# ttwang0303/Adaptive-RGBD-Localization-Mappig

Measured on AMD Instinct MI355X. Metric: frames/sec (extract+match+RANSAC-PnP) @640x480, 2000 kp, higher is better.
Workload: dtype u8/i32 (extract, match), f32+f64 (ransac, pnp)

## Files before the change

adaptive-rgbd-localization-mappig_amd/csrc/k_extract.hip:

```cpp
#include "odo_device.h"
#include "odo_internal.h"
#include "odo_wave.h"
#ifdef FS_STATS
#include <cstdio>
#endif

#ifndef ODO_EXTRACT_PRIO
#define ODO_EXTRACT_PRIO 0
#endif
#define EXTRACT_PRIO() \
    if (ODO_EXTRACT_PRIO) __builtin_amdgcn_s_setprio(ODO_EXTRACT_PRIO)

namespace odo {

__global__ void __launch_bounds__(256) k_gray(const uint8_t* __restrict__ bgr, uint8_t* __restrict__ pyr,
                                              int w, int h, int pitch, size_t in_stride, size_t pyr_stride) {
    EXTRACT_PRIO();
    const int f = blockIdx.y;
    const int q = blockIdx.x * blockDim.x + threadIdx.x;
    const uint8_t* src = bgr + (size_t)f * in_stride;
    uint8_t* dst = pyr + (size_t)f * pyr_stride;
    const int npix = w * h;
    const int p0 = q * 4;
    if (p0 >= npix) return;
// ... 1414 lines not shown
            const int src = reflect101_1(x - 4 + 4 * d + bb, L.w) - (x - 4);
            const int sd = src >> 2, sb = src & 3;
            a |= (uint32_t)(sd == 0 ? sb : sd == 1 ? 4 + sb : 0x0c) << (8 * bb);
            bsel |= (uint32_t)(sd == 2 ? sb : 0x0c) << (8 * bb);
        }
        selA[d] = a;
        selB[d] = bsel;
    }
    const int o0 = x >= 4 ? x - 4 : x, o2 = x + 8 <= L.pitch ? x + 4 : x;
    const uint8_t* s0 = srcL;
    uint8_t* dp = blur + (size_t)f * pyr_stride + L.off + (size_t)y0 * L.pitch + x;
    blur_walk<true, BR_RE>(s0, dp, (size_t)L.pitch, L.h, y0, true, true, true, o0, x, o2, selA, selB);
}

__global__ void __launch_bounds__(256) k_blur_rows(const uint8_t* __restrict__ pyr, uint8_t* __restrict__ blur,
                                                   size_t pyr_stride, const LevelDesc* __restrict__ lv, BlurRows S,
                                                   int nlevels, int eblocks) {
    EXTRACT_PRIO();
    const int f = blockIdx.y;
    if ((int)blockIdx.x < eblocks) {
        const int k = (int)blockIdx.x * 256 + (int)threadIdx.x;
        if (k >= S.ebase[nlevels]) return;
        int l = 0;
        while (l + 1 < nlevels && k >= S.ebase[l + 1]) l++;
        blur_edge_lane(pyr + (size_t)f * pyr_stride + lv[l].off, blur, pyr_stride, lv, S, nlevels, f, k);
        return;
    }
    const uint32_t none[3] = {0, 0, 0};
    const int item = ((int)blockIdx.x - eblocks) * 16 + ((int)threadIdx.x >> 4);
    if (item >= S.base[nlevels]) return;
    int l = 0;
    while (l + 1 < nlevels && item >= S.base[l + 1]) l++;
    const LevelDesc L = lv[l];
    const int it = item - S.base[l];
    const int chunk = it / S.nst[l], strip = it - chunk * S.nst[l];
    const int q = 1 + strip * 16 + ((int)threadIdx.x & 15);
    const bool store = q <= S.nq[l];
    const int x = 4 * (store ? q : S.nq[l]);
    const int y0 = chunk_y0<BR_R>(chunk, L.h);
    const bool top = y0 < 3, bottom = y0 + BR_R + 3 > L.h;
    const uint8_t* s0 = pyr + (size_t)f * pyr_stride + L.off + (x - 4);
    uint8_t* dp = blur + (size_t)f * pyr_stride + L.off + (size_t)y0 * L.pitch + x;
    blur_walk<false, BR_R>(s0, dp, (size_t)L.pitch, L.h, y0, top, bottom, store, 0, 0, 0, none, none);
}

#ifndef PYR_TH
#define PYR_TH 512
#endif
#ifndef PYR_VGPR
#define PYR_ATTR
#else
#define PYR_ATTR __attribute__((amdgpu_waves_per_eu(PYR_VGPR)))
#endif
#ifndef PYR_RU
#define PYR_RU 4
#endif
#ifndef PYR_GU
#define PYR_GU 8
#endif
struct PyrLevels {
    int rx_off[16], ry_off[16];
};
#ifndef PYR_PARTS
#define PYR_PARTS 1
#endif
struct PyrSplit {
    int parts;
    int lo[2][16], hi[2][16], ca[2][16], cb[2][16], ea[2][16], eb[2][16];
};
ODO_INLINE void pyr_blur_level(const uint8_t* srcL, uint8_t* __restrict__ blur, size_t pyr_stride,
                               const LevelDesc* __restrict__ lv, const BlurRows& S, int nlevels, int f, int l,
                               const LevelDesc& L, int t, int ca, int cb, int ea, int eb) {
    const uint32_t none[3] = {0, 0, 0};
    const int items = cb * S.nst[l];
    const int g = t >> 4;
    for (int it = ca * S.nst[l] + g; it < items; it += PYR_TH / 16) {
        const int chunk = it / S.nst[l], strip = it - chunk * S.nst[l];
        const int q = 1 + strip * 16 + (t & 15);
        const bool store = q <= S.nq[l];
        const int x = 4 * (store ? q : S.nq[l]);
        const int y0 = chunk_y0<BR_R>(chunk, L.h);
        const bool top = y0 < 3, bottom = y0 + BR_R + 3 > L.h;
        const uint8_t* s0 = srcL + (x - 4);
        uint8_t* dp = blur + (size_t)f * pyr_stride + L.off + (size_t)y0 * L.pitch + x;
        blur_walk<false, BR_R>(s0, dp, (size_t)L.pitch, L.h, y0, top, bottom, store, 0, 0, 0, none, none);
    }
    const int ne = (S.ebase[l + 1] - S.ebase[l]) / ((L.h + BR_RE - 1) / BR_RE);
    for (int k = S.ebase[l] + ea * ne + t; k < S.ebase[l] + eb * ne; k += PYR_TH)
        blur_edge_lane(srcL, blur, pyr_stride, lv, S, nlevels, f, k);
}
ODO_INLINE void pyr_resize_rows(const uint8_t* srcS, uint8_t* dstD, const LevelDesc& S, const LevelDesc& D,
                                const ResizeX* __restrict__ X, const ResizeY* __restrict__ Y, int t, int ylo, int yhi) {
    const int nq = (D.w + 3) >> 2;
    const int P = PYR_TH / nq;
    if (t >= P * nq) return;
    const int ph = t / nq, q = t - ph * nq;
    const int x00 = X[4 * q].sx0;
    const int wb = x00 & ~3, sh = x00 & 3;
    uint32_t sel[4], wt[4];
#pragma unroll
    for (int j = 0; j < 4; j++) {
        const int dx = 4 * q + j;
        if (dx < D.w) {
            const ResizeX xj = X[dx];
            const uint32_t r0 = (uint32_t)(xj.sx0 - x00), r1 = (uint32_t)(xj.sx1 - x00);
            sel[j] = r0 | (0x0cu << 8) | (r1 << 16) | (0x0cu << 24);
            wt[j] = (uint32_t)xj.a0 | ((uint32_t)xj.a1 << 16);
        } else {
            sel[j] = 0x0c0c0c0cu;
            wt[j] = 0;
        }
    }
    const uint8_t* sbase = srcS + wb;
    uint8_t* dbase = dstD + 4 * q;
    auto hsum = [&](const uint8_t* row, uint32_t (&h)[4]) {
        const uint32_t* w32 = reinterpret_cast<const uint32_t*>(row);
        const uint32_t w0 = w32[0], w1 = w32[1], w2 = w32[2];
        const uint32_t A = __builtin_amdgcn_alignbyte(w1, w0, sh), B = __builtin_amdgcn_alignbyte(w2, w1, sh);
#pragma unroll
        for (int j = 0; j < 4; j++) {
            typedef unsigned short u16x2 __attribute__((ext_vector_type(2)));
            h[j] = __builtin_amdgcn_udot2(__builtin_bit_cast(u16x2, __builtin_amdgcn_perm(B, A, sel[j])),
                                          __builtin_bit_cast(u16x2, wt[j]), 0u, false);
        }
    };
    for (int y = ylo + ph; y < yhi; y += PYR_RU * P) {
        ResizeY Yr[PYR_RU];
#pragma unroll
        for (int u = 0; u < PYR_RU; u++) Yr[u] = Y[min(y + u * P, yhi - 1)];
        uint32_t h0[PYR_RU][4], h1[PYR_RU][4];
#pragma unroll
        for (int u = 0; u < PYR_RU; u++) {
            hsum(sbase + Yr[u].sy0 * S.pitch, h0[u]);
            hsum(sbase + Yr[u].sy1 * S.pitch, h1[u]);
        }
#pragma unroll
        for (int u = 0; u < PYR_RU; u++) {
            uint32_t pk = 0;
#pragma unroll
            for (int j = 0; j < 4; j++)
                pk |= min((__umul24(h0[u][j], (uint32_t)Yr[u].b0) + __umul24(h1[u][j], (uint32_t)Yr[u].b1) + (1u << 21)) >> 22,
                          255u) << (8 * j);
            if (y + u * P < yhi) *reinterpret_cast<uint32_t*>(dbase + (size_t)(y + u * P) * D.pitch) = pk;
        }
    }
}
ODO_INLINE void pyr_gray_rows(const uint8_t* __restrict__ src, uint8_t* gdst, int w, int pitch, int r0, int r1,
                              int t) {
    if ((w & 3) == 0) {
        const int nq4 = (r1 * w) >> 2;
        const int q00 = ((r0 * w) >> 2) + t;
        int cy = (4 * q00) / w, cx = 4 * q00 - cy * w;
        const int dy = (4 * PYR_TH) / w, dx = 4 * PYR_TH - dy * w;
        for (int q0 = q00; q0 < nq4; q0 += PYR_GU * PYR_TH) {
            uint32_t wv[PYR_GU][3];
#pragma unroll
            for (int u = 0; u < PYR_GU; u++) {
                const int q = q0 + u * PYR_TH;
                if (q < nq4) {
                    const uint32_t* s32 = reinterpret_cast<const uint32_t*>(src + (size_t)q * 12);
                    wv[u][0] = s32[0], wv[u][1] = s32[1], wv[u][2] = s32[2];
                }
            }
#pragma unroll
            for (int u = 0; u < PYR_GU; u++) {
                const int q = q0 + u * PYR_TH;
                const int y = cy, x = cx;
                cx += dx;
                cy += dy;
                if (cx >= w) cx -= w, cy++;
                if (q < nq4) {
                    uint32_t out = 0;
#pragma unroll
                    for (int i = 0; i < 4; i++) {
                        const int b = 3 * i;
                        const uint32_t B = (wv[u][b >> 2] >> (8 * (b & 3))) & 0xffu;
                        const uint32_t G = (wv[u][(b + 1) >> 2] >> (8 * ((b + 1) & 3))) & 0xffu;
                        const uint32_t R = (wv[u][(b + 2) >> 2] >> (8 * ((b + 2) & 3))) & 0xffu;
                        out |= ((B * 1868u + G * 9617u + R * 4899u + 8192u) >> 14) << (8 * i);
                    }
                    *reinterpret_cast<uint32_t*>(gdst + (size_t)y * pitch + x) = out;
                }
            }
        }
    } else {
        for (int p = r0 * w + t; p < r1 * w; p += PYR_TH) {
            const uint8_t* s = src + (size_t)p * 3;
            const int yy = p / w, xx = p - yy * w;
            gdst[(size_t)yy * pitch + xx] =
                (uint8_t)(((uint32_t)s[0] * 1868u + (uint32_t)s[1] * 9617u + (uint32_t)s[2] * 4899u + 8192u) >> 14);
        }
    }
}
template <bool BLUR>
__global__ void __launch_bounds__(PYR_TH) PYR_ATTR k_pyramid(const uint8_t* __restrict__ bgr, uint8_t* __restrict__ pyr,
                                                    size_t in_stride, size_t pyr_stride,
                                                    const LevelDesc* __restrict__ lv, const ResizeX* __restrict__ xt,
                                                    const ResizeY* __restrict__ yt, PyrLevels PL, int nlevels,
                                                    uint8_t* __restrict__ blur, BlurRows BR, PyrSplit SP) {
    EXTRACT_PRIO();
    const int part = SP.parts == 2 ? (int)(blockIdx.x & 1) : 0;
    const int f = SP.parts == 2 ? (int)(blockIdx.x >> 1) : (int)blockIdx.x;
    const int t = threadIdx.x;
    uint8_t* base = pyr + (size_t)f * pyr_stride;
    if (bgr) {
        const LevelDesc L0 = lv[0];
        pyr_gray_rows(bgr + (size_t)f * in_stride, base + L0.off, L0.w, L0.pitch, SP.lo[part][0], SP.hi[part][0], t);
    }
    for (int l = 1; l < nlevels; l++) {
        __syncthreads();
        const LevelDesc S = lv[l - 1], D = lv[l];
        if (BLUR)
            pyr_blur_level(base + S.off, blur, pyr_stride, lv, BR, nlevels, f, l - 1, S, t, SP.ca[part][l - 1],
                           SP.cb[part][l - 1], SP.ea[part][l - 1], SP.eb[part][l - 1]);
        pyr_resize_rows(base + S.off, base + D.off, S, D, xt + PL.rx_off[l], yt + PL.ry_off[l], t, SP.lo[part][l],
                        SP.hi[part][l]);
    }
    if (BLUR) {
        __syncthreads();
        const int ll = nlevels - 1;
        const LevelDesc L = lv[ll];
        pyr_blur_level(base + L.off, blur, pyr_stride, lv, BR, nlevels, f, ll, L, t, SP.ca[part][ll], SP.cb[part][ll],
                       SP.ea[part][ll], SP.eb[part][ll]);
    }
    __syncthreads();
}

}

namespace odo {
void launch_gray(hipStream_t st, const uint8_t* bgr, uint8_t* pyr, int w, int h, int pitch, size_t in_stride,
                 size_t pyr_stride, int nframes) {
    dim3 g((w * h / 4 + 255) / 256 + 1, nframes);
    hipLaunchKernelGGL(k_gray, g, dim3(256), 0, st, bgr, pyr, w, h, pitch, in_stride, pyr_stride);
}
static bool blur_rows_plan(const LevelDesc* lv_host, int nlevels, BlurRows& R) {
    bool rows = nlevels <= 16;
    for (int l = 0; l < nlevels; l++) rows = rows && lv_host[l].h >= BR_R && lv_host[l].w >= 12;
    if (!rows) return false;
    R = BlurRows{};
    int acc = 0, eacc = 0;
    for (int l = 0; l < nlevels; l++) {
        const LevelDesc& L = lv_host[l];
        R.base[l] = acc;
        R.ebase[l] = eacc;
        R.nq[l] = (L.w - 8) / 4;
        R.nst[l] = (R.nq[l] + 15) / 16;
        R.nch[l] = (L.h + BR_R - 1) / BR_R;
        acc += R.nst[l] * R.nch[l];
        eacc += (1 + (L.w + 3) / 4 - (R.nq[l] + 1)) * ((L.h + BR_RE - 1) / BR_RE);
    }
    R.base[nlevels] = acc;
    R.ebase[nlevels] = eacc;
    return true;
}
bool pyramid_blur_fusable(const LevelDesc* lv_host, int nlevels) {
    BlurRows R;
    return blur_rows_plan(lv_host, nlevels, R);
}
static void pyramid_split_plan(const LevelDesc* lv_host, const ResizeY* ry_h, const int* ry_off, int nlevels,
                               int parts, PyrSplit& S) {
    S = PyrSplit{};
    S.parts = parts;
    for (int l = 0; l < nlevels && l < 16; l++) {
        const int h = lv_host[l].h, nch = (h + BR_R - 1) / BR_R, nch6 = (h + BR_RE - 1) / BR_RE;
        for (int p = 0; p < 2; p++) {
            S.lo[p][l] = 0, S.hi[p][l] = h;
            S.ca[p][l] = 0, S.cb[p][l] = nch, S.ea[p][l] = 0, S.eb[p][l] = nch6;
        }
    }
    if (parts != 2 || nlevels > 16 || !ry_h) {
        S.parts = 1;
        return;
    }
    int sp[16];
    for (int l = 0; l < nlevels; l++) {
        const int h = lv_host[l].h;
        int s = ((h / 2 + BR_R / 2) / BR_R) * BR_R;
        if (h < 2 * BR_R) s = h;
        s = std::min(s, h < 2 * BR_R ? h : h - BR_R);
        sp[l] = s;
        const int nch = (h + BR_R - 1) / BR_R, nch6 = (h + BR_RE - 1) / BR_RE;
        S.ca[0][l] = 0, S.cb[0][l] = s == h ? nch : s / BR_R;
        S.ca[1][l] = S.cb[0][l], S.cb[1][l] = nch;
        S.ea[0][l] = 0, S.eb[0][l] = s == h ? nch6 : s / BR_RE;
        S.ea[1][l] = S.eb[0][l], S.eb[1][l] = nch6;
    }
    for (int l = nlevels - 1; l >= 0; l--) {
        const int h = lv_host[l].h;
        int thi = std::min(h, sp[l] + 3), blo = std::max(0, sp[l] - 3);
        if (sp[l] == h) blo = h;
        if (l + 1 < nlevels) {
            const ResizeY* Y = ry_h + ry_off[l + 1];
            if (S.hi[0][l + 1] > 0) thi = std::max(thi, Y[S.hi[0][l + 1] - 1].sy1 + 1);
            if (S.lo[1][l + 1] < lv_host[l + 1].h) blo = std::min(blo, Y[S.lo[1][l + 1]].sy0);
        }
        S.lo[0][l] = 0, S.hi[0][l] = std::min(h, thi);
        S.lo[1][l] = std::max(0, blo), S.hi[1][l] = h;
        if (S.lo[1][l] >= h) S.lo[1][l] = h;
    }
}
void launch_pyramid(hipStream_t st, const uint8_t* bgr, uint8_t* pyr, size_t in_stride, size_t pyr_stride,
                    const LevelDesc* lv, const ResizeX* rx, const ResizeY* ry, const int* rx_off, const int* ry_off,
                    int nlevels, int nframes, uint8_t* blur, const LevelDesc* lv_host, const ResizeY* ry_h) {
    PyrLevels PL{};
    for (int l = 0; l < nlevels && l < 16; l++) PL.rx_off[l] = rx_off[l], PL.ry_off[l] = ry_off[l];
    PyrSplit SP;
    pyramid_split_plan(lv_host, ry_h, ry_off, nlevels, PYR_PARTS, SP);
    const dim3 g(nframes * SP.parts);
    BlurRows BR{};
    if (blur && blur_rows_plan(lv_host, nlevels, BR)) {
        hipLaunchKernelGGL(k_pyramid<true>, g, dim3(PYR_TH), 0, st, bgr, pyr, in_stride, pyr_stride, lv, rx, ry, PL,
                           nlevels, blur, BR, SP);
        return;
    }
    hipLaunchKernelGGL(k_pyramid<false>, g, dim3(PYR_TH), 0, st, bgr, pyr, in_stride, pyr_stride, lv, rx, ry, PL,
                       nlevels, (uint8_t*)nullptr, BR, SP);
}
bool pyramid_fusable(const LevelDesc* lv_host, const ResizeX* rx, const int* rx_off, int nlevels) {
    if (nlevels > 16) return false;
    for (int l = 1; l < nlevels; l++) {
        const LevelDesc& D = lv_host[l];
        const int nq = (D.w + 3) / 4;
        if (nq > PYR_TH) return false;
        const ResizeX* X = rx + rx_off[l];
        for (int q = 0; q < nq; q++) {
            const int x00 = X[4 * q].sx0;
            for (int j = 0; j < 4 && 4 * q + j < D.w; j++) {
                const ResizeX& xj = X[4 * q + j];
                if (xj.sx0 < x00 || xj.sx1 < x00 || xj.sx0 - x00 > 7 || xj.sx1 - x00 > 7) return false;
                if (xj.a0 < 0 || xj.a0 > 65535 || xj.a1 < 0 || xj.a1 > 65535) return false;
            }
        }
    }
    return true;
}
size_t resize_lds_bytes(int spitch, int dw, int max_src_rows) {
    return (size_t)((dw + 3) & ~3) * sizeof(ResizeX) + (size_t)max_src_rows * spitch;
}
void launch_resize(hipStream_t st, uint8_t* pyr, size_t pyr_stride, int src_off, int spitch, int dst_off, int dpitch,
                   int dw, int dh, int rb, int max_src_rows, const ResizeX* xt, const ResizeY* yt, int nframes) {
    dim3 g((dh + rb - 1) / rb, nframes);
    const size_t lds = resize_lds_bytes(spitch, dw, max_src_rows);
    hipLaunchKernelGGL(k_resize, g, dim3(256), lds, st, pyr, pyr_stride, src_off, spitch, dst_off, dpitch, dw, dh, rb,
                       xt, yt);
}
bool fast_lds_plan(const FastSeg* segs, int nsegs, FastLds& L) {
    int img = 16, bw = 1, rows = 1, nl = 1;
    for (int k = 0; k < nsegs; k++) {
        img = std::max(img, (int)segs[k].rows * FS_RS);
        bw = std::max(bw, (int)segs[k].rows * (int)segs[k].bw);
        rows = std::max(rows, (int)segs[k].rows);
        nl = std::max(nl, FS_RS / 4 + FS_NCM);
        if ((int)segs[k].ncell > FS_NCM || (int)segs[k].rows * FS_RS > 65536 || ((segs[k].x0 & 15) + segs[k].cols) > FS_RS)
            return false;
    }
    auto al = [](int x) { return (x + 15) & ~15; };
    L.img = al(img);
    L.ring = 2 * L.img;
    L.clist = L.ring + (FS_TH / 64) * FS_RSTRIDE * 2;
    L.bits = al(L.clist + FS_CL * 2);
    L.cnt = al(L.bits + bw * 4);
    L.qlist = al(L.cnt + rows * FS_NCM * 4);
    L.misc = al(L.qlist + nl * 8);
    L.total = al(L.misc + (int)sizeof(FastMisc));
    return L.total <= 160 * 1024;
}
void launch_fast(hipStream_t st, const uint8_t* pyr, size_t pyr_stride, const FastSeg* segs, int nsegs,
                 const LevelDesc* lv, uint32_t* cand, int* cand_cnt, int ncells, int cell_cap, int ini_th, int min_th,
                 const FastLds& lds, int nframes) {
    static bool attr = false;
    if (!attr) {
        (void)hipFuncSetAttribute((const void*)k_fast_seg, hipFuncAttributeMaxDynamicSharedMemorySize, 160 * 1024);
        attr = true;
    }
    hipLaunchKernelGGL(k_fast_seg, dim3(nsegs, nframes), dim3(FS_TH), lds.total, st, pyr, pyr_stride, segs, lv, cand,
                       cand_cnt, ncells, cell_cap, ini_th, min_th, lds);
#ifdef FS_STATS
    unsigned long long h[8];
    (void)hipStreamSynchronize(st);
    (void)hipMemcpyFromSymbol(h, HIP_SYMBOL(fs_stats), sizeof(h));
    fprintf(stderr, "fs_stats frames %d segs %d items0 %llu items1 %llu survivors %llu segtest_calls %llu corners %llu ovf %llu retry_cells %llu cells %llu\n",
            nframes, nsegs, h[0], h[1], h[2], h[3], h[4], h[5], h[6], h[7]);
    static const unsigned long long z[8] = {};
    (void)hipMemcpyToSymbol(HIP_SYMBOL(fs_stats), z, sizeof(z));
// ... 78 lines not shown
```

adaptive-rgbd-localization-mappig_amd/csrc/odo_batch.cpp:

```cpp
#include "odo_ctx.h"

static int wait_pnp_done(odo_ctx* c, hipStream_t st, int set) {
    if (st != c->pdone_st[set]) HIPCHK(hipStreamWaitEvent(st, c->ev_pnp_done[set], 0));
    return ODO_OK;
}

static int queue_batch_waits(odo_ctx* c) {
    int e;
    const int s = next_set(c);
    if (c->pdone_rec[s] && (e = wait_pnp_done(c, c->stream, s))) return e;
    if (c->batch_counter >= (uint64_t)PYR_WAIT && (e = wait_pnp_done(c, c->stream, (s + NSETS - PYR_WAIT) % NSETS)))
        return e;
    return ODO_OK;
}

constexpr int PYR_FUSED_MIN_FRAMES = 128;
static bool build_pyramid(odo_ctx* c, hipStream_t st, const uint8_t* d_bgr, uint8_t* pyr, int n, uint8_t* blur) {
    const size_t P = c->pyr_size;
    const bool fused = c->pyr_fusable && (c->pform == ODO_PYRAMID_FORM_FUSED || c->pform == ODO_PYRAMID_FORM_FUSED_NOBLUR ||
                                          (c->pform == ODO_PYRAMID_FORM_AUTO && n >= PYR_FUSED_MIN_FRAMES));
    if (fused) {
        if (c->pform == ODO_PYRAMID_FORM_FUSED_NOBLUR || !c->blur_fusable) blur = nullptr;
        launch_pyramid(st, d_bgr, pyr, (size_t)c->W * c->H * 3, P, c->lv, c->rx, c->ry, c->rx_off.data(),
                       c->ry_off.data(), c->nlevels, n, blur, c->lv_h.data(),
                       c->ry_h.data());
        return blur != nullptr;
    }
    if (d_bgr) launch_gray(st, d_bgr, pyr, c->W, c->H, c->lv_h[0].pitch, (size_t)c->W * c->H * 3, P, n);
    for (int l = 1; l < c->nlevels; l++) {
        const LevelDesc& S = c->lv_h[l - 1];
        const LevelDesc& D = c->lv_h[l];
        launch_resize(st, pyr, P, S.off, S.pitch, D.off, D.pitch, D.w, D.h, RZ_RB, c->rz_rows[l],
                      c->rx + c->rx_off[l], c->ry + c->ry_off[l], n);
    }
    return false;
}

static int run_extract_adaptive(odo_ctx* c, int set, const uint8_t* d_bgr, const uint16_t* d_depth, int n,
                                int slot0) {
    hipStream_t st = c->stream;
    const size_t P = c->pyr_size;
    const size_t slot = fbase(c, set) + slot0;
    const LevelDesc& L0 = c->lv_h[0];
    uint8_t* pyr = c->pyr + slot * P;
    const size_t nc = (size_t)c->ad_ncells;
    if (d_bgr) launch_gray(st, d_bgr, pyr, c->W, c->H, L0.pitch, (size_t)c->W * c->H * 3, P, n);
    tmark(c, 1, st);
    launch_adapt_smap(st, pyr, P, c->W, c->H, L0.pitch, c->smap, c->smap_stride, n);
    HIPCHK(hipMemsetAsync(c->ahist, 0, (size_t)n * nc * 256 * sizeof(int), st));
    if (c->ad_nbands > 0)
        launch_adapt_cand(st, c->smap, c->smap_stride, L0.pitch, c->adb, c->ad_nbands, c->adc, c->ad_ncells, c->acand,
                          c->acand_stride, c->aband_cnt, c->ahist, n);
    tmark(c, 2, st);
    launch_adapt_chain(st, c->ahist, c->ad_ncells, n, c->cfg.adaptive, c->athresh, c->atsel, c->ansel);
    launch_adapt_select(st, c->acand, c->acand_stride, c->aband_cnt, c->ad_nbands, c->adb, c->adc, c->ad_ncells,
                        c->atsel, c->ansel, c->ad_mpc, c->abig, c->abig_stride, c->acell, c->acell_cnt, n);
    launch_adapt_assemble(st, c->acell, c->acell_cnt, c->ad_ncells, c->ad_mpc, c->cfg.adaptive.retain_best, c->W,
                          c->H, c->akp, c->kp_cap, c->nkp + slot, c->kp_cap, n);
    tmark(c, 3, st);
    launch_blur(st, pyr, c->blur + slot * P, P, c->lv, c->lv_h.data(), 1, n);
    tmark(c, 4, st);
    const FrameSlot f = frame_at(c, slot);
    launch_adapt_finalize(st, c->blur + slot * P, P, L0.pitch, c->akp, c->kp_cap, f.nkp, c->a_cos, c->a_sin, d_depth,
                          (size_t)c->W * c->H, c->W, c->cal, f.kps, f.desc, f.kun, f.xyz, f.ur, c->kp_cap, n);
    tmark(c, 5, st);
    HIPCHK(hipGetLastError());
    return ODO_OK;
}

static int run_extract_adaptive_orb(odo_ctx* c, int set, const uint8_t* d_bgr, const uint16_t* d_depth, int n,
                                    int slot0) {
    hipStream_t st = c->stream;
    const size_t P = c->pyr_size;
    const size_t slot = fbase(c, set) + slot0;
    uint8_t* pyr = c->pyr + slot * P;
    const int nc = c->ad_ncells, ni = (int)c->oai_h.size(), nb = (int)c->oab_h.size();
// ... 398 lines not shown
```

adaptive-rgbd-localization-mappig_amd/csrc/odo_ctx.h:

```cpp
#pragma once

#include <hip/hip_runtime.h>

#include <algorithm>
#include <cmath>
#include <cstdio>
#include <cstdlib>
#include <cstring>
#include <string>
#include <vector>

#include "../../include/odo.h"
#include "odo_device.h"
#include "odo_internal.h"

namespace odo {

extern thread_local std::string g_err;
inline int fail(int code, const std::string& msg) {
    g_err = msg;
    return code;
}

#define HIPCHK(x)                                                                                   \
// ... 81 lines not shown
        cap = 0;
    }
    int reserve(size_t bytes, size_t floor, const char* who) {
        if (bytes <= cap) return ODO_OK;
        release();
        const size_t want = std::max(bytes, floor);
        if ((PINNED ? hipHostMalloc((void**)&p, want, hipHostMallocDefault) : hipMalloc((void**)&p, want)) != hipSuccess) {
            p = nullptr;
            (void)hipGetLastError();
            return fail(ODO_ERR_DEVICE, std::string(who) + (PINNED ? ": hipHostMalloc failed" : ": hipMalloc failed"));
        }
        cap = want;
        return ODO_OK;
    }
};
using DevBlock = GrowBlock<false>;
using PinnedBlock = GrowBlock<true>;

struct HypSession;
void free_hyp_session(HypSession* h);

}

using namespace odo;
struct odo_ctx {
    odo_config cfg{};
    HypSession* hs = nullptr;
    DevPool pool;
    std::vector<hipEvent_t> events;
    hipError_t make_event(hipEvent_t* e, unsigned flags) {
        const hipError_t r = hipEventCreateWithFlags(e, flags);
        if (r == hipSuccess) events.push_back(*e);
        return r;
    }
    int device = 0;
    hipStream_t stream = nullptr;
    hipStream_t pstream = nullptr, pstream2 = nullptr;
    std::vector<hipStream_t> owned;
    hipEvent_t ev_latch = nullptr;
    bool latch_rec = false;
    hipEvent_t ev_geo[NSETS] = {};
    bool geo_rec[NSETS] = {};
    uint64_t batch_counter = 0;
    int W = 0, H = 0, maxb = 0, slots = 0, nlevels = 0;
    std::vector<LevelDesc> lv_h;
    std::vector<CellDesc> cells_h;
    std::vector<int> rx_off, ry_off, rz_rows;
    int pform = ODO_PYRAMID_FORM_AUTO;
    bool pyr_fusable = false, blur_fusable = false;
    LevelDesc* lv = nullptr;
    CellDesc* cells = nullptr;
    ResizeX* rx = nullptr;
    ResizeY* ry = nullptr;
    std::vector<ResizeY> ry_h;
    int ncells = 0, cell_cap = 0, kp_cap = 0, okp_stride = 0, node_cap = 0, match_cap = 0, mask_words = 0;
    int max_blur_tiles = 0;
    int fast_roi = 0;
    std::vector<FastSeg> fsegs_h;
    FastSeg* fsegs = nullptr;
    FastLds fs_lds{};
    size_t pyr_size = 0, keys_per_frame = 0;
    FrameCalib cal{};
    RansacCfg rcfg{};
    uint8_t *pyr = nullptr, *blur = nullptr;
    uint32_t* cand = nullptr;
    int* cand_cnt = nullptr;
    uint32_t* keys = nullptr;
    int32_t* knode = nullptr;
    uint32_t* okp = nullptr;
    int* ocnt = nullptr;
    orb_kp* kps = nullptr;
    uint8_t* desc = nullptr;
    float *kun = nullptr, *xyz = nullptr, *ur = nullptr;
    int* nkp = nullptr;
    uint8_t* bgr_in[2] = {};
    uint16_t* depth_in[2] = {};
    hipStream_t cstream = nullptr;
    hipEvent_t ev_in_copied[2] = {}, ev_in_free[2] = {};
    bool in_used[2] = {};
    hipEvent_t ev_depth_done = nullptr;
    bool depth_busy = false;
    PinnedBlock stage;
    DevArena hyp_arena;
    PinnedBlock hyp_stage;
    hipEvent_t hyp_up = nullptr;
    bool hyp_up_rec = false;
    int in_next = 0;
    int2 *knn_idx[NSETS] = {}, *knn_dist[NSETS] = {};
    uint32_t* lm_bits[NSETS] = {};
    int32_t* qlist[NSETS] = {};
    int* qcnt[NSETS] = {};
    int lm_words = 0;
    int knn_split = 2;
    bool knn_mx = true;
    int last_knn_set = -1, last_knn_n = 0;
    uint64_t* sort_scratch = nullptr;
    double* latch = nullptr;
    void* rscr[NSETS] = {};
    struct PairBufs {
        odo_dmatch* matches = nullptr;
        int *n_matches = nullptr, *n_good = nullptr, *pair_valid = nullptr;
        void* good = nullptr;
        int32_t* f2_src = nullptr;
        uint32_t* best_mask = nullptr;
        odo_pair_result* res = nullptr;
        float* T12 = nullptr;
// ... 194 lines not shown
```

adaptive-rgbd-localization-mappig_amd/csrc/odo_geometry.cpp:

```cpp
#include "odo_ctx.h"

inline int cvRoundH(float v) { return (int)lrintf(v); }
inline int cvFloorH(float v) {
    int i = (int)v;
    return i - (i > v);
}
inline int satShort(float v) {
    int r = cvRoundH(v);
    return std::min(std::max(r, -32768), 32767);
}

static int build_adaptive_orb_geometry(odo_ctx* c) {
    const odo_adaptive_params& P = c->cfg.adaptive;
    float scale[OA_NLEV];
    int quota[OA_NLEV];
    {
        const double sf = (double)1.2f;
        const float factor = (float)(1.0 / sf);
        float nd = 10000 * (1 - factor) / (1 - (float)pow((double)factor, (double)OA_NLEV));
        int sum = 0;
        for (int l = 0; l < OA_NLEV; l++) {
            scale[l] = (float)pow(sf, (double)l);
            c->osc.s[l] = scale[l];
            if (l < OA_NLEV - 1) {
// ... 300 lines not shown
            int sx = cvFloorH(fx);
            fx -= sx;
            if (sx < 0) {
                fx = 0;
                sx = 0;
            }
            if (sx + 1 >= S.w) {
                xmax = std::min(xmax, dx);
                if (sx >= S.w - 1) {
                    fx = 0;
                    sx = S.w - 1;
                }
            }
            xofs[dx] = sx;
            a0[dx] = satShort((1.f - fx) * 2048);
            a1[dx] = satShort(fx * 2048);
        }
        for (int dx = 0; dx < D.w; dx++) {
            ResizeX X;
            X.sx0 = xofs[dx];
            if (dx < xmax) {
                X.sx1 = xofs[dx] + 1;
                X.a0 = a0[dx];
                X.a1 = a1[dx];
            } else {
                X.sx1 = xofs[dx];
                X.a0 = 2048;
                X.a1 = 0;
            }
            rx.push_back(X);
        }
        c->ry_off[l] = (int)ry.size();
        for (int dy = 0; dy < D.h; dy++) {
            float fy = (float)((dy + 0.5) * scale_y - 0.5);
            int sy = cvFloorH(fy);
            fy -= sy;
            ResizeY Y;
            Y.b0 = satShort((1.f - fy) * 2048);
            Y.b1 = satShort(fy * 2048);
            Y.sy0 = std::min(std::max(sy, 0), S.h - 1);
            Y.sy1 = std::min(std::max(sy + 1, 0), S.h - 1);
            ry.push_back(Y);
        }
        int mr = 1;
        for (int y0 = 0; y0 < D.h; y0 += RZ_RB) {
            const int y1 = std::min(y0 + RZ_RB, D.h) - 1;
            mr = std::max(mr, ry[c->ry_off[l] + y1].sy1 - ry[c->ry_off[l] + y0].sy0 + 1);
        }
        c->rz_rows[l] = mr;
        if (resize_lds_bytes(S.pitch, D.w, mr) > 64 * 1024) return fail(ODO_ERR_ARG, "image too wide for the resize band");
    }
    c->pform = c->cfg.forms.pyramid;
    if (const char* e = odo_knob("ODO_PYRAMID_FORM")) c->pform = atoi(e);
    c->pyr_fusable = pyramid_fusable(c->lv_h.data(), rx.data(), c->rx_off.data(), p.nlevels);
    c->blur_fusable = c->pyr_fusable && pyramid_blur_fusable(c->lv_h.data(), p.nlevels);
    int e;
    if ((e = c->pool.alloc(&c->lv, c->lv_h.size()))) return e;
    if ((e = c->pool.alloc(&c->cells, c->cells_h.size()))) return e;
    if ((e = c->pool.alloc(&c->rx, rx.size()))) return e;
    if ((e = c->pool.alloc(&c->ry, ry.size()))) return e;
    HIPCHK(hipMemcpy(c->lv, c->lv_h.data(), c->lv_h.size() * sizeof(LevelDesc), hipMemcpyHostToDevice));
    HIPCHK(hipMemcpy(c->cells, c->cells_h.data(), c->cells_h.size() * sizeof(CellDesc), hipMemcpyHostToDevice));
    if (!fast_lds_plan(c->fsegs_h.data(), (int)c->fsegs_h.size(), c->fs_lds))
        return fail(ODO_ERR_ARG, "FAST segments exceed LDS");
    if ((e = c->pool.alloc(&c->fsegs, std::max<size_t>(c->fsegs_h.size(), 1)))) return e;
    if (!c->fsegs_h.empty())
        HIPCHK(hipMemcpy(c->fsegs, c->fsegs_h.data(), c->fsegs_h.size() * sizeof(FastSeg), hipMemcpyHostToDevice));
    if (!rx.empty()) HIPCHK(hipMemcpy(c->rx, rx.data(), rx.size() * sizeof(ResizeX), hipMemcpyHostToDevice));
    if (!ry.empty()) HIPCHK(hipMemcpy(c->ry, ry.data(), ry.size() * sizeof(ResizeY), hipMemcpyHostToDevice));
    c->ry_h = ry;
    return ODO_OK;
}
```

adaptive-rgbd-localization-mappig_amd/csrc/odo_internal.h:

```cpp
#pragma once

#include <hip/hip_runtime.h>
#include <stddef.h>
#include <stdint.h>
#include <stdlib.h>

#include "../../include/odo_types.h"

namespace odo {

static inline const char* odo_knob(const char* name) {
#ifdef ODO_TUNING
    return getenv(name);
#else
    (void)name;
    return nullptr;
#endif
}

struct Pack {
    size_t off = 0;
    size_t add(size_t bytes) {
        const size_t o = off;
        off = (off + bytes + 255) & ~(size_t)255;
// ... 6 lines not shown
struct LevelDesc {
    int off;
    int w, h;
    int pitch;
    float scale;
    int quota;
    int cell_begin;
    int cell_end;
    int key_off;
};

struct CellDesc {
    int16_t level;
    int16_t rows, cols;
    int16_t x0, y0;
    int16_t offx, offy;
    int16_t pad;
};

#ifndef FS_SEGC
#define FS_SEGC 8
#endif
#define FS_NCM FS_SEGC
#ifndef FS_RS
#define FS_RS 272
#endif
struct FastSeg {
    int level, ci0;
    int16_t y0, x0, rows, cols, ncell, wcell;
    int16_t bw;
    int16_t nw, rstep, rmag;
    float inv_w;
};
static_assert(sizeof(FastSeg) == 32, "FastSeg is read as two uint4");
inline void fast_seg_staging(FastSeg& G) {
    const int nw = ((G.x0 & 15) + G.cols + 15) >> 4;
    G.nw = (int16_t)nw;
    G.rstep = (int16_t)(256 / nw);
    G.rmag = (int16_t)((4096 + nw - 1) / nw);
    G.inv_w = 1.0f / (float)G.wcell;
}
struct FastLds {
    int img;
    int ring, clist, bits, cnt, qlist, misc, total;
};

struct ResizeX {
    int sx0, sx1;
    int a0, a1;
};
struct ResizeY {
    int sy0, sy1;
    int b0, b1;
};

struct FrameCalib {
    float fx, fy, cx, cy;
    float k1, k2, p1, p2, k3;
    float depth_factor, mbf;
    float invfx, invfy;
};

__device__ inline void kp_geometry(float uu, float vv, const FrameCalib& cal, const uint16_t* depth, int img_w,
                                   float* ku, float* p3, float* urp) {
    float ux = uu, uy = vv;
    if (cal.k1 != 0.0f) {
        const double fx = cal.fx, fy = cal.fy, cx = cal.cx, cy = cal.cy;
        const double ifx = 1. / fx, ify = 1. / fy;
        const double k0 = cal.k1, k1 = cal.k2, k2 = cal.p1, k3 = cal.p2, k4 = cal.k3;
        double x = uu, y = vv;
        x = (x - cx) * ifx;
        y = (y - cy) * ify;
        const double x0 = x, y0 = y;
        for (int j = 0; j < 5; j++) {
            double r2 = x * x + y * y;
            double icdist = 1 / (1 + ((k4 * r2 + k1) * r2 + k0) * r2);
            double deltaX = 2 * k2 * x * y + k3 * (r2 + 2 * x * x);
            double deltaY = k2 * (r2 + 2 * y * y) + 2 * k3 * x * y;
            x = (x0 - deltaX) * icdist;
            y = (y0 - deltaY) * icdist;
        }
        ux = (float)(fx * x + cx);
        uy = (float)(fy * y + cy);
    }
    ku[0] = ux;
    ku[1] = uy;
    float urv = -1.f, X = 0.f, Y = 0.f, Z = 0.f;
    const uint16_t d16 = depth[(size_t)((int)vv) * img_w + (int)uu];
    const float z = (float)d16 * cal.depth_factor + 0.0f;
    if (z > 0) {
        urv = ux - cal.mbf / z;
        X = (ux - cal.cx) * z * cal.invfx;
        Y = (uy - cal.cy) * z * cal.invfy;
        Z = z;
    }
    p3[0] = X;
    p3[1] = Y;
    p3[2] = Z;
    *urp = urv;
}

#define AD_BH 16
#define AD_MAXW 1024
#define AD_SEL_LDS 4096
using AdParams = odo_adaptive_params;

// ... 1 lines not shown
    int rs, re, cs, ce;
    int r0, r1, c0, c1;
    int band0, band1;
    int cand_cap;
    int pad;
};
struct AdBand {
    int cell, y0, y1, cand_off;
};

#define OA_NLEV 8
#define OA_EDGE 15
#define OA_PATCH 31
#ifndef OA_BH
#define OA_BH 64
#endif
struct OaImg {
    int off, w, h, pitch;
    int quota;
    int band0, band1;
    int cand_cap;
};
struct OaCell {
    int rs, cs, cw, ch;
    int img0;
    int pad[3];
};
struct OaBand {
    int img, y0, y1, cand_off;
};
struct OaScales {
    float s[OA_NLEV];
};

struct RansacCfg {
    int iterations;
    int min_inlier_th;
    float max_mahal;
    int sample_size;
    int check_depth;
    double raster_cov_x, raster_cov_y;
    int h0;
    int lanes_min_open;
    int fold_wave;
    int first_hyps;
};

void launch_kp_geometry(hipStream_t st, const orb_kp* kps, const int* nkp, const uint16_t* depth, size_t depth_stride,
                        int img_w, FrameCalib cal, float* kun, float* xyz, float* ur, int kp_cap, int nframes);
void launch_gray(hipStream_t st, const uint8_t* bgr, uint8_t* pyr, int w, int h, int pitch, size_t in_stride,
                 size_t pyr_stride, int nframes);
size_t resize_lds_bytes(int spitch, int dw, int max_src_rows);
void launch_pyramid(hipStream_t st, const uint8_t* bgr, uint8_t* pyr, size_t in_stride, size_t pyr_stride,
                    const LevelDesc* lv, const ResizeX* rx, const ResizeY* ry, const int* rx_off, const int* ry_off,
                    int nlevels, int nframes, uint8_t* blur, const LevelDesc* lv_host,
                    const ResizeY* ry_h);
bool pyramid_blur_fusable(const LevelDesc* lv_host, int nlevels);
bool pyramid_fusable(const LevelDesc* lv_host, const ResizeX* rx, const int* rx_off, int nlevels);
void launch_resize(hipStream_t st, uint8_t* pyr, size_t pyr_stride, int src_off, int spitch, int dst_off, int dpitch,
                   int dw, int dh, int rb, int max_src_rows, const ResizeX* xt, const ResizeY* yt, int nframes);
void launch_fast(hipStream_t st, const uint8_t* pyr, size_t pyr_stride, const FastSeg* segs, int nsegs,
                 const LevelDesc* lv, uint32_t* cand, int* cand_cnt, int ncells, int cell_cap, int ini_th, int min_th,
                 const FastLds& lds, int nframes);
bool fast_lds_plan(const FastSeg* segs, int nsegs, FastLds& L);
size_t octree_lds_bytes(int node_cap);
void launch_octree(hipStream_t st, const uint32_t* cand, const int* cand_cnt, const LevelDesc* lv, int ncells,
                   int cell_cap, int nlevels, uint32_t* keys, int32_t* knode, size_t keys_stride,
                   uint32_t* okp, int* ocnt, int okp_stride, int node_cap, int nframes);
void launch_blur(hipStream_t st, const uint8_t* pyr, uint8_t* blur, size_t pyr_stride, const LevelDesc* lv,
                 const LevelDesc* lv_host, int nlevels, int nframes);
void launch_finalize(hipStream_t st, const uint8_t* pyr, const uint8_t* blur, size_t pyr_stride, const LevelDesc* lv,
                     int nlevels, const uint32_t* okp, const int* ocnt, int okp_stride, const uint16_t* depth,
                     size_t depth_stride, int img_w, FrameCalib cal, orb_kp* kps, uint8_t* desc, float* kun, float* xyz,
                     float* ur, int* nkp, int kp_cap, int nframes, bool geometry = true);
void launch_pair_valid(hipStream_t st, int* pv, int n, int first_valid);
void launch_copy_frame(hipStream_t st, const orb_kp* kps_s, const uint8_t* desc_s, const float* kun_s,
                       const float* xyz_s, const float* ur_s, const int* n_s, orb_kp* kps_d, uint8_t* desc_d,
                       float* kun_d, float* xyz_d, float* ur_d, int* n_d, int kp_cap);
void launch_knn2(hipStream_t st, const uint8_t* q, const int* qn, size_t q_stride, const uint8_t* t, const int* tn,
                 size_t t_stride, int2* idx, int2* dist, size_t out_stride, int max_q, int npairs,
                 const int32_t* qlist = nullptr, const int* qcnt = nullptr, size_t ql_stride = 0, int nsplit = 1,
                 size_t split_stride = 0);
void launch_knn2_f4(hipStream_t st, const uint8_t* q, const int* qn, size_t q_stride, const uint8_t* t, const int* tn,
                    size_t t_stride, int2* idx, int2* dist, size_t out_stride, int max_q, int npairs,
                    const int32_t* qlist = nullptr, const int* qcnt = nullptr, size_t ql_stride = 0);
void launch_vo_lm(hipStream_t st, const float* xyz, const int* nkp, int kp_cap, int slot0, float th_depth_m,
                  uint32_t* lm_bits, int lm_words, int32_t* qlist, int* qcnt, int npairs);
void launch_pair_match(hipStream_t st, const int2* knn_idx, const int2* knn_dist, size_t knn_stride, const float* xyz,
                       const int* nkp, int kp_cap, int slot0, float ratio, const uint32_t* lm_bits, int lm_words,
                       int nsplit, size_t split_stride, int check_depth,
                       odo_dmatch* matches, int* n_matches, void* good, int* n_good, int32_t* f2_src,
                       uint64_t* sort_scratch, int match_cap, int npairs);
int launch_sort_dbg(hipStream_t st, void* a, int n);
void launch_latch(hipStream_t st, double* latch, const void* good, const int* n_good, const int* n_matches,
                  const odo_dmatch* matches, const float* xyz, int kp_cap, int slot0, int npairs, int match_cap,
                  int min_inl, int sample_size, int iterations, const int* pair_valid, int* set_flag = nullptr);
size_t ransac_gpt_bytes();
void launch_ransac_raw(hipStream_t st, void* scratch, int npairs, int match_cap, int mask_words, RansacCfg cfg,
                       uint64_t seed_base, uint64_t pair_base, odo_rng* rng_io);
void launch_ransac(hipStream_t st, const void* good, const int* n_good, const int* n_matches,
                   const odo_dmatch* matches, const float* xyz, int kp_cap, int slot0, int match_cap, RansacCfg cfg,
                   const double* latch, const int* pair_valid, int min_matches, odo_rng* rng_io, void* scratch,
                   uint32_t* best_mask, int mask_words, odo_pair_result* res, float* T12, int npairs,
                   int* open_hint = nullptr);
void launch_ransac_hyps(hipStream_t st, const void* good, const int* n_good, const int* n_matches,
                        const odo_dmatch* matches, const float* xyz, int kp_cap, int slot0, int match_cap,
                        RansacCfg cfg, const double* latch, const int* pair_valid, int min_matches, odo_rng* rng_io,
                        void* scratch, uint32_t* best_mask, int mask_words, odo_pair_result* res, float* T12,
                        int npairs, int h_lo, int h_hi);
size_t ransac_scratch_bytes(int npairs, int match_cap, int mask_words, const RansacCfg& cfg);
void ransac_read_hyps(hipStream_t st, void* scratch, int match_cap, int mask_words, RansacCfg cfg, int h0, int h1,
// ... 238 lines not shown
```

Before: 165,700.

## Restructure fused pyramid resize for row reuse, 8-wide outputs and LDS row tables

```diff
diff --git a/adaptive-rgbd-localization-mappig_amd/csrc/k_extract.hip b/adaptive-rgbd-localization-mappig_amd/csrc/k_extract.hip
--- a/adaptive-rgbd-localization-mappig_amd/csrc/k_extract.hip
+++ b/adaptive-rgbd-localization-mappig_amd/csrc/k_extract.hip
@@ -1490,14 +1490,16 @@
 #else
 #define PYR_ATTR __attribute__((amdgpu_waves_per_eu(PYR_VGPR)))
 #endif
-#ifndef PYR_RU
-#define PYR_RU 4
+#ifndef PYR_RQ
+#define PYR_RQ 4
 #endif
+#define PYR_YCAP 2048
 #ifndef PYR_GU
 #define PYR_GU 8
 #endif
 struct PyrLevels {
     int rx_off[16], ry_off[16];
+    int ycap;
 };
 #ifndef PYR_PARTS
 #define PYR_PARTS 1
@@ -1528,20 +1530,26 @@
         blur_edge_lane(srcL, blur, pyr_stride, lv, S, nlevels, f, k);
 }
 ODO_INLINE void pyr_resize_rows(const uint8_t* srcS, uint8_t* dstD, const LevelDesc& S, const LevelDesc& D,
-                                const ResizeX* __restrict__ X, const ResizeY* __restrict__ Y, int t, int ylo, int yhi) {
-    const int nq = (D.w + 3) >> 2;
-    const int P = PYR_TH / nq;
-    if (t >= P * nq) return;
-    const int ph = t / nq, q = t - ph * nq;
-    const int x00 = X[4 * q].sx0;
-    const int wb = x00 & ~3, sh = x00 & 3;
-    uint32_t sel[4], wt[4];
-#pragma unroll
-    for (int j = 0; j < 4; j++) {
-        const int dx = 4 * q + j;
+                                const ResizeX* __restrict__ X, const ResizeYP* Y, int t, int ylo, int yhi) {
+    const int no = (D.w + 7) >> 3;
+    const int nb = PYR_TH / no;
+    if (t >= nb * no) return;
+    const int bk = t / no, q = t - bk * no;
+    const int rb = (yhi - ylo + nb - 1) / nb;
+    const int ya = ylo + bk * rb, n = min(ya + rb, yhi) - ya;
+    if (n <= 0) return;
+    const int x00 = X[8 * q].sx0;
+    const int x04 = 8 * q + 4 < D.w ? X[8 * q + 4].sx0 : x00 + 4;
+    const int wb = x00 & ~3;
+    const uint32_t sh = (uint32_t)(x00 & 3), sh2 = (uint32_t)(x04 - x00 - 4);
+    uint32_t sel[8], wt[8];
+#pragma unroll
+    for (int j = 0; j < 8; j++) {
+        const int dx = 8 * q + j;
         if (dx < D.w) {
             const ResizeX xj = X[dx];
-            const uint32_t r0 = (uint32_t)(xj.sx0 - x00), r1 = (uint32_t)(xj.sx1 - x00);
+            const int o = j < 4 ? x00 : x04;
+            const uint32_t r0 = (uint32_t)(xj.sx0 - o), r1 = (uint32_t)(xj.sx1 - o);
             sel[j] = r0 | (0x0cu << 8) | (r1 << 16) | (0x0cu << 24);
             wt[j] = (uint32_t)xj.a0 | ((uint32_t)xj.a1 << 16);
         } else {
@@ -1549,37 +1557,62 @@
             wt[j] = 0;
         }
     }
-    const uint8_t* sbase = srcS + wb;
-    uint8_t* dbase = dstD + 4 * q;
-    auto hsum = [&](const uint8_t* row, uint32_t (&h)[4]) {
-        const uint32_t* w32 = reinterpret_cast<const uint32_t*>(row);
-        const uint32_t w0 = w32[0], w1 = w32[1], w2 = w32[2];
-        const uint32_t A = __builtin_amdgcn_alignbyte(w1, w0, sh), B = __builtin_amdgcn_alignbyte(w2, w1, sh);
-#pragma unroll
-        for (int j = 0; j < 4; j++) {
-            typedef unsigned short u16x2 __attribute__((ext_vector_type(2)));
-            h[j] = __builtin_amdgcn_udot2(__builtin_bit_cast(u16x2, __builtin_amdgcn_perm(B, A, sel[j])),
-                                          __builtin_bit_cast(u16x2, wt[j]), 0u, false);
-        }
+    const uint32_t spitch = (uint32_t)S.pitch;
+    auto load_row = [&](uint32_t (&w)[4], uint32_t row) {
+        const uint32_t* w32 = reinterpret_cast<const uint32_t*>(srcS + (row * spitch + (uint32_t)wb));
+        w[0] = w32[0], w[1] = w32[1], w[2] = w32[2], w[3] = w32[3];
     };
-    for (int y = ylo + ph; y < yhi; y += PYR_RU * P) {
-        ResizeY Yr[PYR_RU];
-#pragma unroll
-        for (int u = 0; u < PYR_RU; u++) Yr[u] = Y[min(y + u * P, yhi - 1)];
-        uint32_t h0[PYR_RU][4], h1[PYR_RU][4];
-#pragma unroll
-        for (int u = 0; u < PYR_RU; u++) {
-            hsum(sbase + Yr[u].sy0 * S.pitch, h0[u]);
-            hsum(sbase + Yr[u].sy1 * S.pitch, h1[u]);
-        }
-#pragma unroll
-        for (int u = 0; u < PYR_RU; u++) {
-            uint32_t pk = 0;
-#pragma unroll
-            for (int j = 0; j < 4; j++)
-                pk |= min((__umul24(h0[u][j], (uint32_t)Yr[u].b0) + __umul24(h1[u][j], (uint32_t)Yr[u].b1) + (1u << 21)) >> 22,
-                          255u) << (8 * j);
-            if (y + u * P < yhi) *reinterpret_cast<uint32_t*>(dbase + (size_t)(y + u * P) * D.pitch) = pk;
+    auto windows = [&](const uint32_t (&w)[4], uint32_t (&W)[4]) {
+        const uint32_t A1 = __builtin_amdgcn_alignbyte(w[2], w[1], sh), A2 = __builtin_amdgcn_alignbyte(w[3], w[2], sh);
+        const uint32_t A3 = __builtin_amdgcn_alignbyte(0u, w[3], sh);
+        W[0] = __builtin_amdgcn_alignbyte(w[1], w[0], sh);
+        W[1] = A1;
+        W[2] = __builtin_amdgcn_alignbyte(A2, A1, sh2);
+        W[3] = __builtin_amdgcn_alignbyte(A3, A2, sh2);
+    };
+    auto hpix = [&](const uint32_t (&W)[4], int j) {
+        typedef unsigned short u16x2 __attribute__((ext_vector_type(2)));
+        const uint32_t p = j < 4 ? __builtin_amdgcn_perm(W[1], W[0], sel[j]) : __builtin_amdgcn_perm(W[3], W[2], sel[j]);
+        return __builtin_amdgcn_udot2(__builtin_bit_cast(u16x2, p), __builtin_bit_cast(u16x2, wt[j]), 0u, false);
+    };
+    const ResizeYP* Yp = Y + ya;
+    uint32_t dof = (uint32_t)ya * (uint32_t)D.pitch + 8u * (uint32_t)q;
+    uint32_t rq[PYR_RQ][4];
+#pragma unroll
+    for (int u = 0; u < PYR_RQ; u++) load_row(rq[u], Yp[min(u, n - 1)].rows >> 16);
+    ResizeYP Ye = Yp[0];
+    uint32_t x0[4];
+    load_row(x0, Ye.rows & 0xffffu);
+    uint32_t held[8] = {}, heldrow = ~0u;
+    for (int i = 0; i < n; i += PYR_RQ) {
+#pragma unroll
+        for (int u = 0; u < PYR_RQ; u++) {
+            const int k = i + u;
+            const ResizeYP Yn = Yp[min(k + 1, n - 1)];
+            const uint32_t rfill = Yp[min(k + PYR_RQ, n - 1)].rows >> 16;
+            const uint32_t r0 = Ye.rows & 0xffffu, r1 = Ye.rows >> 16;
+            if (r0 != heldrow) {
+                uint32_t W[4];
+                windows(x0, W);
+#pragma unroll
+                for (int j = 0; j < 8; j++) held[j] = hpix(W, j);
+            }
+            if ((Yn.rows & 0xffffu) != r1) load_row(x0, Yn.rows & 0xffffu);
+            uint32_t W[4];
+            windows(rq[u], W);
+            load_row(rq[u], rfill);
+            const uint32_t b0 = Ye.wts & 0xffffu, b1 = Ye.wts >> 16;
+            uint32_t pk[2] = {0, 0};
+#pragma unroll
+            for (int j = 0; j < 8; j++) {
+                const uint32_t h1 = hpix(W, j);
+                pk[j >> 2] |= min((__umul24(held[j], b0) + __umul24(h1, b1) + (1u << 21)) >> 22, 255u) << (8 * (j & 3));
+                held[j] = h1;
+            }
+            *reinterpret_cast<uint2*>(dstD + dof) = make_uint2(pk[0], pk[1]);
+            dof += k + 1 < n ? (uint32_t)D.pitch : 0u;
+            heldrow = r1;
+            Ye = Yn;
         }
     }
 }
@@ -1634,25 +1667,27 @@
 __global__ void __launch_bounds__(PYR_TH) PYR_ATTR k_pyramid(const uint8_t* __restrict__ bgr, uint8_t* __restrict__ pyr,
                                                     size_t in_stride, size_t pyr_stride,
                                                     const LevelDesc* __restrict__ lv, const ResizeX* __restrict__ xt,
-                                                    const ResizeY* __restrict__ yt, PyrLevels PL, int nlevels,
+                                                    const ResizeYP* __restrict__ yt, PyrLevels PL, int nlevels,
                                                     uint8_t* __restrict__ blur, BlurRows BR, PyrSplit SP) {
     EXTRACT_PRIO();
     const int part = SP.parts == 2 ? (int)(blockIdx.x & 1) : 0;
     const int f = SP.parts == 2 ? (int)(blockIdx.x >> 1) : (int)blockIdx.x;
     const int t = threadIdx.x;
     uint8_t* base = pyr + (size_t)f * pyr_stride;
+    extern __shared__ ResizeYP ylds[];
     if (bgr) {
         const LevelDesc L0 = lv[0];
         pyr_gray_rows(bgr + (size_t)f * in_stride, base + L0.off, L0.w, L0.pitch, SP.lo[part][0], SP.hi[part][0], t);
     }
     for (int l = 1; l < nlevels; l++) {
+        const LevelDesc S = lv[l - 1], D = lv[l];
+        ResizeYP* yl = ylds + (l & 1) * PL.ycap;
+        for (int i = t; i < D.h; i += PYR_TH) yl[i] = yt[PL.ry_off[l] + i];
         __syncthreads();
-        const LevelDesc S = lv[l - 1], D = lv[l];
         if (BLUR)
             pyr_blur_level(base + S.off, blur, pyr_stride, lv, BR, nlevels, f, l - 1, S, t, SP.ca[part][l - 1],
                            SP.cb[part][l - 1], SP.ea[part][l - 1], SP.eb[part][l - 1]);
-        pyr_resize_rows(base + S.off, base + D.off, S, D, xt + PL.rx_off[l], yt + PL.ry_off[l], t, SP.lo[part][l],
-                        SP.hi[part][l]);
+        pyr_resize_rows(base + S.off, base + D.off, S, D, xt + PL.rx_off[l], yl, t, SP.lo[part][l], SP.hi[part][l]);
     }
     if (BLUR) {
         __syncthreads();
@@ -1739,36 +1774,44 @@
     }
 }
 void launch_pyramid(hipStream_t st, const uint8_t* bgr, uint8_t* pyr, size_t in_stride, size_t pyr_stride,
-                    const LevelDesc* lv, const ResizeX* rx, const ResizeY* ry, const int* rx_off, const int* ry_off,
+                    const LevelDesc* lv, const ResizeX* rx, const ResizeYP* ry, const int* rx_off, const int* ry_off,
                     int nlevels, int nframes, uint8_t* blur, const LevelDesc* lv_host, const ResizeY* ry_h) {
     PyrLevels PL{};
     for (int l = 0; l < nlevels && l < 16; l++) PL.rx_off[l] = rx_off[l], PL.ry_off[l] = ry_off[l];
+    for (int l = 1; l < nlevels && l < 16; l++) PL.ycap = std::max(PL.ycap, lv_host[l].h);
+    const size_t lds = 2 * (size_t)PL.ycap * sizeof(ResizeYP);
     PyrSplit SP;
     pyramid_split_plan(lv_host, ry_h, ry_off, nlevels, PYR_PARTS, SP);
     const dim3 g(nframes * SP.parts);
     BlurRows BR{};
     if (blur && blur_rows_plan(lv_host, nlevels, BR)) {
-        hipLaunchKernelGGL(k_pyramid<true>, g, dim3(PYR_TH), 0, st, bgr, pyr, in_stride, pyr_stride, lv, rx, ry, PL,
+        hipLaunchKernelGGL(k_pyramid<true>, g, dim3(PYR_TH), lds, st, bgr, pyr, in_stride, pyr_stride, lv, rx, ry, PL,
                            nlevels, blur, BR, SP);
         return;
     }
-    hipLaunchKernelGGL(k_pyramid<false>, g, dim3(PYR_TH), 0, st, bgr, pyr, in_stride, pyr_stride, lv, rx, ry, PL,
+    hipLaunchKernelGGL(k_pyramid<false>, g, dim3(PYR_TH), lds, st, bgr, pyr, in_stride, pyr_stride, lv, rx, ry, PL,
                        nlevels, (uint8_t*)nullptr, BR, SP);
 }
-bool pyramid_fusable(const LevelDesc* lv_host, const ResizeX* rx, const int* rx_off, int nlevels) {
+bool pyramid_fusable(const LevelDesc* lv_host, const ResizeX* rx, const int* rx_off, int nlevels, size_t pyr_size) {
     if (nlevels > 16) return false;
     for (int l = 1; l < nlevels; l++) {
+        const LevelDesc& S = lv_host[l - 1];
         const LevelDesc& D = lv_host[l];
-        const int nq = (D.w + 3) / 4;
-        if (nq > PYR_TH) return false;
+        const int no = (D.w + 7) / 8;
+        if (no > PYR_TH || S.h > 65536 || D.h > PYR_YCAP) return false;
         const ResizeX* X = rx + rx_off[l];
-        for (int q = 0; q < nq; q++) {
-            const int x00 = X[4 * q].sx0;
-            for (int j = 0; j < 4 && 4 * q + j < D.w; j++) {
-                const ResizeX& xj = X[4 * q + j];
-                if (xj.sx0 < x00 || xj.sx1 < x00 || xj.sx0 - x00 > 7 || xj.sx1 - x00 > 7) return false;
+        for (int q = 0; q < no; q++) {
+            const int x00 = X[8 * q].sx0, wb = x00 & ~3;
+            const int x04 = 8 * q + 4 < D.w ? X[8 * q + 4].sx0 : x00 + 4;
+            if (wb < 0 || x04 - x00 < 4 || x04 - x00 > 7) return false;
+            for (int j = 0; j < 8 && 8 * q + j < D.w; j++) {
+                const ResizeX& xj = X[8 * q + j];
+                const int o = j < 4 ? x00 : x04;
+                if (xj.sx0 < o || xj.sx1 < o || xj.sx0 - o > 7 || xj.sx1 - o > 7) return false;
+                if (xj.sx0 - wb > 15 || xj.sx1 - wb > 15) return false;
                 if (xj.a0 < 0 || xj.a0 > 65535 || xj.a1 < 0 || xj.a1 > 65535) return false;
             }
+            if ((size_t)S.off + (size_t)(S.h - 1) * S.pitch + wb + 16 > pyr_size) return false;
         }
     }
     return true;
diff --git a/adaptive-rgbd-localization-mappig_amd/csrc/odo_batch.cpp b/adaptive-rgbd-localization-mappig_amd/csrc/odo_batch.cpp
--- a/adaptive-rgbd-localization-mappig_amd/csrc/odo_batch.cpp
+++ b/adaptive-rgbd-localization-mappig_amd/csrc/odo_batch.cpp
@@ -21,7 +21,7 @@
                                           (c->pform == ODO_PYRAMID_FORM_AUTO && n >= PYR_FUSED_MIN_FRAMES));
     if (fused) {
         if (c->pform == ODO_PYRAMID_FORM_FUSED_NOBLUR || !c->blur_fusable) blur = nullptr;
-        launch_pyramid(st, d_bgr, pyr, (size_t)c->W * c->H * 3, P, c->lv, c->rx, c->ry, c->rx_off.data(),
+        launch_pyramid(st, d_bgr, pyr, (size_t)c->W * c->H * 3, P, c->lv, c->rx, c->ryp, c->rx_off.data(),
                        c->ry_off.data(), c->nlevels, n, blur, c->lv_h.data(),
                        c->ry_h.data());
         return blur != nullptr;
diff --git a/adaptive-rgbd-localization-mappig_amd/csrc/odo_ctx.h b/adaptive-rgbd-localization-mappig_amd/csrc/odo_ctx.h
--- a/adaptive-rgbd-localization-mappig_amd/csrc/odo_ctx.h
+++ b/adaptive-rgbd-localization-mappig_amd/csrc/odo_ctx.h
@@ -157,6 +157,7 @@
     CellDesc* cells = nullptr;
     ResizeX* rx = nullptr;
     ResizeY* ry = nullptr;
+    ResizeYP* ryp = nullptr;
     std::vector<ResizeY> ry_h;
     int ncells = 0, cell_cap = 0, kp_cap = 0, okp_stride = 0, node_cap = 0, match_cap = 0, mask_words = 0;
     int max_blur_tiles = 0;
diff --git a/adaptive-rgbd-localization-mappig_amd/csrc/odo_geometry.cpp b/adaptive-rgbd-localization-mappig_amd/csrc/odo_geometry.cpp
--- a/adaptive-rgbd-localization-mappig_amd/csrc/odo_geometry.cpp
+++ b/adaptive-rgbd-localization-mappig_amd/csrc/odo_geometry.cpp
@@ -376,13 +376,22 @@
     }
     c->pform = c->cfg.forms.pyramid;
     if (const char* e = odo_knob("ODO_PYRAMID_FORM")) c->pform = atoi(e);
-    c->pyr_fusable = pyramid_fusable(c->lv_h.data(), rx.data(), c->rx_off.data(), p.nlevels);
+    c->pyr_fusable = pyramid_fusable(c->lv_h.data(), rx.data(), c->rx_off.data(), p.nlevels, c->pyr_size);
     c->blur_fusable = c->pyr_fusable && pyramid_blur_fusable(c->lv_h.data(), p.nlevels);
+    std::vector<ResizeYP> ryp(ry.size());
+    for (size_t i = 0; i < ry.size(); i++) {
+        const ResizeY& Y = ry[i];
+        if (Y.sy0 > 65535 || Y.sy1 > 65535 || Y.b0 < 0 || Y.b0 > 65535 || Y.b1 < 0 || Y.b1 > 65535)
+            c->pyr_fusable = c->blur_fusable = false;
+        ryp[i].rows = (uint32_t)Y.sy0 | ((uint32_t)Y.sy1 << 16);
+        ryp[i].wts = (uint32_t)Y.b0 | ((uint32_t)Y.b1 << 16);
+    }
     int e;
     if ((e = c->pool.alloc(&c->lv, c->lv_h.size()))) return e;
     if ((e = c->pool.alloc(&c->cells, c->cells_h.size()))) return e;
     if ((e = c->pool.alloc(&c->rx, rx.size()))) return e;
     if ((e = c->pool.alloc(&c->ry, ry.size()))) return e;
+    if ((e = c->pool.alloc(&c->ryp, ryp.size()))) return e;
     HIPCHK(hipMemcpy(c->lv, c->lv_h.data(), c->lv_h.size() * sizeof(LevelDesc), hipMemcpyHostToDevice));
     HIPCHK(hipMemcpy(c->cells, c->cells_h.data(), c->cells_h.size() * sizeof(CellDesc), hipMemcpyHostToDevice));
     if (!fast_lds_plan(c->fsegs_h.data(), (int)c->fsegs_h.size(), c->fs_lds))
@@ -392,6 +401,7 @@
         HIPCHK(hipMemcpy(c->fsegs, c->fsegs_h.data(), c->fsegs_h.size() * sizeof(FastSeg), hipMemcpyHostToDevice));
     if (!rx.empty()) HIPCHK(hipMemcpy(c->rx, rx.data(), rx.size() * sizeof(ResizeX), hipMemcpyHostToDevice));
     if (!ry.empty()) HIPCHK(hipMemcpy(c->ry, ry.data(), ry.size() * sizeof(ResizeY), hipMemcpyHostToDevice));
+    if (!ryp.empty()) HIPCHK(hipMemcpy(c->ryp, ryp.data(), ryp.size() * sizeof(ResizeYP), hipMemcpyHostToDevice));
     c->ry_h = ry;
     return ODO_OK;
 }
diff --git a/adaptive-rgbd-localization-mappig_amd/csrc/odo_internal.h b/adaptive-rgbd-localization-mappig_amd/csrc/odo_internal.h
--- a/adaptive-rgbd-localization-mappig_amd/csrc/odo_internal.h
+++ b/adaptive-rgbd-localization-mappig_amd/csrc/odo_internal.h
@@ -82,6 +82,9 @@
 struct ResizeY {
     int sy0, sy1;
     int b0, b1;
+};
+struct ResizeYP {
+    uint32_t rows, wts;
 };
 
 struct FrameCalib {
@@ -189,11 +192,11 @@
                  size_t pyr_stride, int nframes);
 size_t resize_lds_bytes(int spitch, int dw, int max_src_rows);
 void launch_pyramid(hipStream_t st, const uint8_t* bgr, uint8_t* pyr, size_t in_stride, size_t pyr_stride,
-                    const LevelDesc* lv, const ResizeX* rx, const ResizeY* ry, const int* rx_off, const int* ry_off,
+                    const LevelDesc* lv, const ResizeX* rx, const ResizeYP* ryp, const int* rx_off, const int* ry_off,
                     int nlevels, int nframes, uint8_t* blur, const LevelDesc* lv_host,
                     const ResizeY* ry_h);
 bool pyramid_blur_fusable(const LevelDesc* lv_host, int nlevels);
-bool pyramid_fusable(const LevelDesc* lv_host, const ResizeX* rx, const int* rx_off, int nlevels);
+bool pyramid_fusable(const LevelDesc* lv_host, const ResizeX* rx, const int* rx_off, int nlevels, size_t pyr_size);
 void launch_resize(hipStream_t st, uint8_t* pyr, size_t pyr_stride, int src_off, int spitch, int dst_off, int dpitch,
                    int dw, int dh, int rb, int max_src_rows, const ResizeX* xt, const ResizeY* yt, int nframes);
 void launch_fast(hipStream_t st, const uint8_t* pyr, size_t pyr_stride, const FastSeg* segs, int nsegs,
```

Measured after the change: 167,100 (median of 3 runs). Within noise of the previous version (+0.8%).
